# thegedge/StereoReconstruction

Hardware: AMD Instinct MI355X
Metric: Mdisparity-hypotheses/s (WxHxD) (higher is better)
Workload: dtype f64; 1 GPU; C3: synthetic rectified 1920x1080 pair, 256 depth levels, GeodesicWeight r=5; TwoView WTA both directions + cross-check; one pair per GPU; width=1920, height=1080, depth_levels=256, window_radius=5, weights=geodesic, pairs_per_gpu=1, pair_seed_rank0=1592590339, pair_seed_of_rank_r=seed + 0x10000*r, parallelism=single GPU

## Files before the change

stereoreconstruction_amd/csrc/srh_strip.hip:

```cpp
#include "srh_internal.hpp"
#include "srh_geom.hpp"
#include "srh_walk.hpp"

#include <type_traits>

namespace srh {

#ifdef SRH_EXPERIMENT
__device__ int g_strip_exp_repeat = 1;
void strip_exp_set(int repeat) { (void)hipMemcpyToSymbol(HIP_SYMBOL(g_strip_exp_repeat), &repeat, sizeof(int)); }
#endif

#define ST_TP 32
#define ST_NCB 8
#define ST_CHUNK 320
#define ST_BROWS 1

typedef __attribute__((address_space(3))) void st_lds_void;
typedef __attribute__((address_space(1))) const void st_gbl_void;
typedef __attribute__((address_space(3))) volatile int st_lds_vint;

__global__ void padded_plane_kernel(const double *__restrict__ gray_tv, int W, int H, double *__restrict__ out)
{
	const int SP = padded_stride(W), HP = H + 2*SRH_PADY;
	const size_t n = (size_t)SP*HP;
	const double nan = __builtin_nan("");
	for (size_t k = (size_t)blockIdx.x*blockDim.x + threadIdx.x; k < n; k += (size_t)gridDim.x*blockDim.x) {
		const int x = (int)(k % (size_t)SP) - SRH_PADL, y = (int)(k / (size_t)SP) - SRH_PADY;
		out[k] = (x >= 0 && y >= 0 && x < W && y < H) ? gray_tv[(size_t)y*W + x] : nan;
	}
}

void launch_padded_plane(hipStream_t st, const double *gray_tv, int w, int h, double *out) {
	size_t n = padded_size(w, h);
	size_t b = (n + 255)/256; if (b > 4096) b = 4096;
	hipLaunchKernelGGL(padded_plane_kernel, dim3((unsigned)b), dim3(256), 0, st, gray_tv, w, h, out);
}

__global__ void padded_full_kernel(const double *__restrict__ gray_tv, int W, int H, int R, uint8_t *__restrict__ out)
{
	const int SP = padded_stride(W), HP = H + 2*SRH_PADY;
	const size_t n = (size_t)SP*HP;
	for (size_t k = (size_t)blockIdx.x*blockDim.x + threadIdx.x; k < n; k += (size_t)gridDim.x*blockDim.x) {
		const int x = (int)(k % (size_t)SP) - SRH_PADL, y = (int)(k / (size_t)SP) - SRH_PADY;
		bool ok = x - R >= 0 && y - R >= 0 && x + R < W && y + R < H;
		for (int row = -R; ok && row <= R; ++row)
			for (int col = -R; col <= R; ++col) {
				const double v = gray_tv[(size_t)(y + row)*W + (x + col)];
				ok = ok && (v == v);
			}
		out[k] = ok ? 1 : 0;
	}
}

void launch_padded_full(hipStream_t st, const double *gray_tv, int w, int h, int R, uint8_t *out) {
	size_t n = padded_size(w, h);
	size_t b = (n + 255)/256; if (b > 4096) b = 4096;
	hipLaunchKernelGGL(padded_full_kernel, dim3((unsigned)b), dim3(256), 0, st, gray_tv, w, h, R, out);
}

__global__ void pixel_range_kernel(const ViewDev *__restrict__ views, int ref, int oth, srh_params P, int y0, int nrows,
                                   const double *__restrict__ tnum, int cstride, PixRange *__restrict__ prange)
{
	const ViewDev &L = views[ref];
	const int W = L.w;
	const size_t q = (size_t)blockIdx.x*blockDim.x + threadIdx.x;
	if (q >= (size_t)nrows*W) return;
	const int x = (int)(q % W), y = y0 + (int)(q / W);
	int lo = 0, hi = -1;
	if (L.mask[(size_t)y*W + x] == 1) {
		const Ray ray = cam_unproject(L.cam, (x + 0.5) / P.image_scale, (y + 0.5) / P.image_scale);
		pinhole_column_range(ray, L.cam, views[oth], P, tnum, cstride, lo, hi);
	}
	PixRange r; r.lo = lo; r.hi = hi;
	prange[q] = r;
}

void launch_pixel_range(hipStream_t st, const ViewDev *views, int ref, int oth, int width, const srh_params &P,
                        int y0, int nrows, const double *tnum, int cstride, PixRange *prange)
{
	const size_t n = (size_t)nrows*width;
	hipLaunchKernelGGL(pixel_range_kernel, dim3((unsigned)((n + 255)/256)), dim3(256), 0, st,
	                   views, ref, oth, P, y0, nrows, tnum, cstride, prange);
}

int strip_chunk_columns() { return ST_CHUNK; }

struct StripArgs {
	int W, H, y0, nrows;
	const double *wimg;
	const double *pconst;
	const PixRange *prange;
	const double *ref_tvp, *oth_tvp;
	const uint8_t *oth_fullp;
	double *cost; int cstride;
	Counters *cnt;
	int n1, n2;
	int nitems;
	double weight_cutoff, bad_ret, max_color_diff;
	CertBound cb;
	int redo;
};

static void strip_items(StripArgs &a) {
	a.n1 = ((a.nrows*3/4)/16)*16;
	a.n2 = a.n1 + (((a.nrows - a.n1)*2/3)/8)*8;
	const int nseg = a.n1/16 + (a.n2 - a.n1)/8 + (a.nrows - a.n2 + 3)/4;
	a.nitems = nseg*((a.W + ST_TP - 1)/ST_TP);
}

template <int R, int NBUF>
struct StripSmem {
	static constexpr int WS = 2*R + 1;
	static constexpr int T = WS*WS;
	static constexpr int WP = (WS + 1) & ~1;
	static constexpr int WPIX = WS*WP;
	static constexpr int RW = ST_CHUNK + 2*R + ST_NCB + 2;
	static constexpr int LW = (ST_TP + 2*R + 1) & ~1;
	static constexpr int NS = WS + 1;
	static constexpr int FW = (RW + 4 + 15) & ~15;
	static constexpr int NBMAX = ST_CHUNK/ST_NCB + 1;
	static constexpr int GL_CAP = 3072;
	static constexpr int GL_SINGLES = GL_CAP - ST_TP*NBMAX;
	alignas(16) double w[NBUF][WS][ST_TP][WP];
	alignas(16) double rt[NS][RW];
	alignas(16) double rto[NBUF == 2 ? NS : 1][RW];
	alignas(16) double lt[NS][LW];
	alignas(16) double pc[2][ST_TP][SRH_PC];
	alignas(16) PixRange pr[2][ST_TP];
	alignas(16) unsigned char full[2][FW];
	unsigned short glist[GL_CAP];
	int glist_n, gsingle_n;
	int item;
	unsigned long long badcols[ST_CHUNK/64 + 2];
	int simd[8];
	int prog[NBUF == 2 ? 8 : 1][64];
	static_assert(ST_CHUNK <= 512 && ST_TP <= 64, "work-list entry = pixel*512 + column in 16 bits");
	static_assert(RW % 2 == 0 && LW % 2 == 0 && WP % 2 == 0, "16-byte rows");
	static_assert(RW - R + 4 <= SRH_PADR + 1, "padded planes cover every staged piece");
};

__device__ __forceinline__ void st_dma16(const void *src, void *dst, int nbytes, int lane) {
	for (int off = 0; off < nbytes; off += 1024) {
		if (off + lane*16 < nbytes)
			__builtin_amdgcn_global_load_lds((st_gbl_void *)((const char *)src + off + lane*16),
			                                 (st_lds_void *)((char *)dst + off), 16, 0, 0);
	}
}
__device__ __forceinline__ void st_dma4(const void *src, void *dst, int nbytes, int lane) {
	for (int off = 0; off < nbytes; off += 256) {
		if (off + lane*4 < nbytes)
			__builtin_amdgcn_global_load_lds((st_gbl_void *)((const char *)src + off + lane*4),
			                                 (st_lds_void *)((char *)dst + off), 4, 0, 0);
	}
}

template <int R, int NBUF>
__device__ __noinline__ double strip_cost_general(const StripSmem<R, NBUF> &S, int wb, int s0, int i, int rc,
                                                  double weight_cutoff, double bad_ret, double max_color_diff)
{
	typedef StripSmem<R, NBUF> Smem;
	constexpr int WS = Smem::WS, NS = Smem::NS;
	double meanL = 0, meanR = 0, totalWeight = 0.0;
#pragma unroll 1
	for (int row = 0; row < WS; ++row) {
		const int sl = s0 + row >= NS ? s0 + row - NS : s0 + row;
		double gl[WS], gr[WS], wt[WS];
#pragma unroll
		for (int col = 0; col < WS; ++col) { gl[col] = S.lt[sl][i + col]; gr[col] = S.rt[sl][rc + col]; wt[col] = S.w[wb][row][i][col]; }
#pragma unroll
		for (int col = 0; col < WS; ++col) {
			const bool ok = gl[col] == gl[col] && gr[col] == gr[col] && wt[col] > weight_cutoff;
			const double pl = wt[col]*gl[col], pr = wt[col]*gr[col];
			meanL += ok ? pl : 0.0;
			meanR += ok ? pr : 0.0;
			totalWeight += ok ? wt[col] : 0.0;
		}
	}
	if (totalWeight < 1e-10) return bad_ret;
	meanL /= totalWeight;
	meanR /= totalWeight;
	double sum1 = 0, sum2 = 0, sum3 = 0;
#pragma unroll 1
	for (int row = 0; row < WS; ++row) {
		const int sl = s0 + row >= NS ? s0 + row - NS : s0 + row;
		double gl[WS], gr[WS], wt[WS];
#pragma unroll
		for (int col = 0; col < WS; ++col) { gl[col] = S.lt[sl][i + col]; gr[col] = S.rt[sl][rc + col]; wt[col] = S.w[wb][row][i][col]; }
#pragma unroll
		for (int col = 0; col < WS; ++col) {
			const bool ok = gl[col] == gl[col] && gr[col] == gr[col] && wt[col] > weight_cutoff;
			const double a = wt[col]*gl[col] - meanL;
			const double b = wt[col]*gr[col] - meanR;
			const double ab = a*b, aa = a*a, bb = b*b;
			sum1 += ok ? ab : 0.0;
			sum2 += ok ? aa : 0.0;
			sum3 += ok ? bb : 0.0;
		}
	}
	const double v = 255*(1.0 - fabs(sum1) / sqrt(sum2 * sum3));
	return (v < max_color_diff) ? v : max_color_diff;
}

template <int R, int NBUF>
__device__ __noinline__ void strip_select_block(const StripSmem<R, NBUF> &S, int wb, int s0, int pi, int rc, unsigned store,
                                                double *__restrict__ dst, double weight_cutoff, double bad_ret, double max_color_diff,
                                                int ra, int rb)
{
	typedef StripSmem<R, NBUF> Smem;
	constexpr int WS = Smem::WS, NS = Smem::NS, NCB = ST_NCB, NR = NCB + 2*R;
	double mLs[NCB], mRs[NCB], tws[NCB];
#pragma unroll
	for (int j = 0; j < NCB; ++j) { mLs[j] = 0.0; mRs[j] = 0.0; tws[j] = 0.0; }
#pragma unroll 1
	for (int row = ra; row < rb; ++row) {
		const int sl = s0 + row >= NS ? s0 + row - NS : s0 + row;
		double rr[NR], rv[NR];
		const double2 *rp = reinterpret_cast<const double2 *>((NBUF == 2 && (rc & 1)) ? &S.rto[sl][rc - 1] : &S.rt[sl][rc]);
#pragma unroll
		for (int m = 0; m < NR/2; ++m) { const double2 v = rp[m]; rr[2*m] = v.x; rr[2*m + 1] = v.y; }
#pragma unroll
		for (int m = 0; m < NR; ++m) { const bool okr = rr[m] == rr[m]; rv[m] = okr ? 1.0 : 0.0; rr[m] = okr ? rr[m] : 0.0; }
#pragma unroll
		for (int col = 0; col < WS; ++col) {
			const double gl = S.lt[sl][pi + col], wt = S.w[wb][row][pi][col];
			const bool okl = gl == gl && wt > weight_cutoff;
			const double w0 = okl ? wt : 0.0, pl0 = okl ? wt*gl : 0.0;
#pragma unroll
			for (int j = 0; j < NCB; ++j) {
				mLs[j] += pl0*rv[col + j];
				mRs[j] += w0*rr[col + j];
				tws[j] += w0*rv[col + j];
			}
		}
	}
#pragma unroll
	for (int j = 0; j < NCB; ++j) { mLs[j] /= tws[j]; mRs[j] /= tws[j]; }
	double s1[NCB], s2v[NCB], s3[NCB];
#pragma unroll
	for (int j = 0; j < NCB; ++j) { s1[j] = 0.0; s2v[j] = 0.0; s3[j] = 0.0; }
#pragma unroll 1
	for (int row = ra; row < rb; ++row) {
		const int sl = s0 + row >= NS ? s0 + row - NS : s0 + row;
		double rr[NR], rv[NR];
		const double2 *rp = reinterpret_cast<const double2 *>((NBUF == 2 && (rc & 1)) ? &S.rto[sl][rc - 1] : &S.rt[sl][rc]);
#pragma unroll
		for (int m = 0; m < NR/2; ++m) { const double2 v = rp[m]; rr[2*m] = v.x; rr[2*m + 1] = v.y; }
#pragma unroll
		for (int m = 0; m < NR; ++m) { const bool okr = rr[m] == rr[m]; rv[m] = okr ? 1.0 : 0.0; rr[m] = okr ? rr[m] : 0.0; }
#pragma unroll
		for (int col = 0; col < WS; ++col) {
			const double gl = S.lt[sl][pi + col], wt = S.w[wb][row][pi][col];
			const bool okl = gl == gl && wt > weight_cutoff;
			const double pl = wt*(gl == gl ? gl : 0.0), kl = okl ? 1.0 : 0.0;
#pragma unroll
			for (int j = 0; j < NCB; ++j) {
				const double k = kl*rv[col + j];
				const double a = (pl - mLs[j])*k, bq = (wt*rr[col + j] - mRs[j])*k;
				s1[j] += a*bq;
				s2v[j] += a*a;
				s3[j] += bq*bq;
			}
		}
	}
#pragma unroll
	for (int j = 0; j < NCB; ++j) {
		if ((store >> j) & 1u) {
			double result = bad_ret;
			if (!(tws[j] < 1e-10)) {
				const double v = 255*(1.0 - fabs(s1[j]) / sqrt(s2v[j] * s3[j]));
				result = (v < max_color_diff) ? v : max_color_diff;
			}
			dst[(ptrdiff_t)j*ST_TP] = result;
		}
	}
}

template <int R, int NWV, int NBUF, int AR, bool BORDER>
__global__ __launch_bounds__(NWV*64, 2)
void twoview_strip_cost_kernel(const StripArgs A)
{
	constexpr bool FMA = AR != 0, CERT = AR == 3 || AR == 5, ONEPASS = AR == 5;
	typedef StripSmem<R, NBUF> Smem;
	constexpr int WS = Smem::WS, WP = Smem::WP, WPIX = Smem::WPIX, RW = Smem::RW, LW = Smem::LW, NS = Smem::NS;
	constexpr int NCB = ST_NCB, CHUNK = ST_CHUNK;
	constexpr int NR = NCB + 2*R;
	constexpr int G = 2*NWV;
	constexpr int NT = NWV*64;
	constexpr bool PAD = NBUF == 1;
	static_assert(NR % 2 == 0, "16-byte rows");
	static_assert((NWV == 4 && NBUF == 1) || (NWV == 8 && NBUF == 2), "two forms");
	extern __shared__ __align__(16) unsigned char smem_raw[];
	Smem &S = *reinterpret_cast<Smem *>(smem_raw);
	const Smem &CS = S;

	const int tid = threadIdx.x;
	const int lane = tid & 63;
	const int wv = __builtin_amdgcn_readfirstlane(tid >> 6);
	const int pg = wv & 3;
	const int i = pg*8 + (lane & 7);
	const int g = (lane >> 3) + 8*(wv >> 2);
	const int W = A.W;
	const int tiles_per_row = (W + ST_TP - 1)/ST_TP;
	const int SP = padded_stride(W);
	unsigned n_dev = 0;
	int partner = wv;
	if (NWV == 8) {
		const int simd = (int)__builtin_amdgcn_s_getreg((1 << 11) | (4 << 6) | 4);
		if (lane == 0) S.simd[wv] = simd;
		S.prog[wv][lane] = 0;
		__syncthreads();
		for (int j = 0; j < NWV; ++j) if (j != wv && CS.simd[j] == simd) { partner = j; break; }
		partner = __builtin_amdgcn_readfirstlane(partner);
	}
	int prog = 0;
	auto prog_step = [&](int units, int &seen) {
		if (NWV == 8) {
			prog += units;
			*(st_lds_vint *)&S.prog[wv][lane] = prog;
			seen = *(st_lds_vint *)&S.prog[partner][lane];
		}
	};
	auto prog_yield = [&](int seen) {
		if (NWV == 8) {
			const int ps = __builtin_amdgcn_readfirstlane(seen), pm = __builtin_amdgcn_readfirstlane(prog);
			asm volatile("s_nop 0\n\ts_cmp_gt_i32 %0, %1\n\ts_cbranch_scc1 1f\n\ts_setprio 1\n\ts_branch 2f\n1:\n\ts_setprio 0\n2:"
			             :: "s"(pm), "s"(ps) : "scc");
		}
	};
#ifdef SRH_PROFILE_PHASES
	unsigned long long ph[8] = {0, 0, 0, 0, 0, 0, 0, 0};
	unsigned long long tp = __builtin_readcyclecounter();
	const unsigned long long t_begin = tp;
	unsigned long long n_tiles = 0, n_gen = 0;
#define ST_STAMP(k) do { const unsigned long long tn_ = __builtin_readcyclecounter(); ph[k] += tn_ - tp; tp = tn_; } while (0)
#else
#define ST_STAMP(k) do { } while (0)
#endif

	for (;;) {
		if (tid == 0) S.item = (int)atomicAdd(BORDER ? &A.cnt->strip_ticket_border : &A.cnt->strip_ticket, 1u);
		__syncthreads();
		const int item = __builtin_amdgcn_readfirstlane(S.item);
		ST_STAMP(0);
		if (item >= A.nitems) break;
		int seg = item / tiles_per_row, tx = item - seg*tiles_per_row;
		if (BORDER) {
			const int nseg = (A.n1 + ST_BROWS - 1)/ST_BROWS + (A.nrows - A.n2 + ST_BROWS - 1)/ST_BROWS;
			const int k = item / nseg;
			seg = item - k*nseg;
			tx = k == 0 ? 0 : k == 1 ? tiles_per_row - 1 : k - 1;
		}
		int ya, nh;
		if (BORDER) {
			const int st = (A.n1 + ST_BROWS - 1)/ST_BROWS;
			if (seg < st) { ya = seg*ST_BROWS; nh = A.n1 - ya; }
			else { ya = A.n2 + (seg - st)*ST_BROWS; nh = A.nrows - ya; }
			if (nh > ST_BROWS) nh = ST_BROWS;
		} else {
			const int s16 = A.n1 >> 4, s8 = (A.n2 - A.n1) >> 3;
			if (seg < s16) { ya = seg*16; nh = 16; }
			else if (seg < s16 + s8) { ya = A.n1 + (seg - s16)*8; nh = 8; }
			else { ya = A.n2 + (seg - s16 - s8)*4; nh = 4; }
			if (ya + nh > A.nrows) nh = A.nrows - ya;
		}
		const int x0 = tx*ST_TP;
		const int x = x0 + i;
		int cs = 0, rowbase = 0;

		auto issue_tile_inputs = [&](int r, int buf, int wb, bool consts, bool windows) {
			const size_t px0 = (size_t)r*W + x0;
			if (consts && wv == 0) st_dma16(A.pconst + px0*SRH_PC, &S.pc[buf][0][0], ST_TP*SRH_PC*8, lane);
			if (consts && wv == 1) st_dma4(A.prange + px0, &S.pr[buf][0], ST_TP*8, lane);
			if (windows) {
				const double *wt = A.wimg + ((size_t)r*tiles_per_row + tx)*(size_t)(ST_TP*WPIX);
				if (NBUF == 1) {
					for (int a = 0; a < WS; ++a)
						st_dma16(wt + (size_t)a*(ST_TP*WP) + pg*8*WP, &S.w[wb][a][pg*8][0], 8*WP*8, lane);
				} else {
					constexpr int NBYTES = ST_TP*WPIX*8;
					for (int off = wv*1024; off < NBYTES; off += NWV*1024)
						if (off + lane*16 < NBYTES)
							__builtin_amdgcn_global_load_lds((st_gbl_void *)((const char *)wt + off + lane*16),
							                                 (st_lds_void *)((char *)&S.w[wb][0][0][0] + off), 16, 0, 0);
				}
			}
		};
		auto issue_row = [&](int yy, int sl) {
			const double *src = A.oth_tvp + (size_t)(yy + SRH_PADY)*SP + (cs - R + SRH_PADL);
			if (wv < 3) { if (wv*1024 + lane*16 < RW*8) __builtin_amdgcn_global_load_lds((st_gbl_void *)((const char *)src + wv*1024 + lane*16),
			                                                                              (st_lds_void *)((char *)&S.rt[sl][0] + wv*1024), 16, 0, 0); }
			else if (wv == 3) st_dma16(A.ref_tvp + (size_t)(yy + SRH_PADY)*SP + (x0 - R + SRH_PADL), &S.lt[sl][0], LW*8, lane);
			else if (NBUF == 2 && wv < 7) {
				const int pc = wv - 4;
				if (pc*1024 + lane*16 < RW*8) __builtin_amdgcn_global_load_lds((st_gbl_void *)((const char *)(src + 1) + pc*1024 + lane*16),
				                                                                (st_lds_void *)((char *)&S.rto[sl][0] + pc*1024), 16, 0, 0);
			}
		};
		static_assert(RW*8 <= 3*1024, "three pieces per row of the other view");
		auto issue_full = [&](int fy, int fb) {
			const size_t a0 = (size_t)(fy + SRH_PADY)*SP + (size_t)(cs + SRH_PADL);
			if (!BORDER && wv == NWV - 1) st_dma4(A.oth_fullp + (a0 & ~(size_t)3), &S.full[fb][0], (RW + 4 + 3) & ~3, lane);
		};

		bool first = true;
		for (int r = ya; r < ya + nh; ++r) {
			const int y = A.y0 + r;
			const int cur = (r - ya) & 1, nxt = cur ^ 1;
			const int wcur = NBUF == 2 ? cur : 0, wnxt = NBUF == 2 ? nxt : 0;
			const bool has_next = r + 1 < ya + nh;
			if (first) issue_tile_inputs(r, cur, wcur, true, true);
			asm volatile("s_waitcnt vmcnt(0)" ::: "memory");
			ST_STAMP(1);
			__builtin_amdgcn_s_barrier();
			ST_STAMP(2);

			int cmin, cmax, cmin_raw;
			{
				const int pi = lane & 31;
				const PixRange q = CS.pr[cur][pi];
				int lo = q.lo, hi = q.hi;
				if (x0 + pi >= W) { lo = 0; hi = -1; }
				if (hi >= lo) hi = dense_cover_hi(lo, hi, NCB, G, PAD);
				int mn = hi >= lo ? lo : 2147483647, mx = hi >= lo ? hi : -2147483647;
#define ST_ROR(v, n) __builtin_amdgcn_update_dpp(0, (v), 0x120 + (n), 0xf, 0xf, false)
#pragma unroll
				for (int d = 8; d >= 1; d >>= 1) {
					const int on = d == 8 ? ST_ROR(mn, 8) : d == 4 ? ST_ROR(mn, 4) : d == 2 ? ST_ROR(mn, 2) : ST_ROR(mn, 1);
					const int ox = d == 8 ? ST_ROR(mx, 8) : d == 4 ? ST_ROR(mx, 4) : d == 2 ? ST_ROR(mx, 2) : ST_ROR(mx, 1);
					mn = on < mn ? on : mn; mx = ox > mx ? ox : mx;
				}
#undef ST_ROR
				{
					const int m0 = __builtin_amdgcn_readlane(mn, 0), m1 = __builtin_amdgcn_readlane(mn, 16);
					const int x0_ = __builtin_amdgcn_readlane(mx, 0), x1_ = __builtin_amdgcn_readlane(mx, 16);
					cmin_raw = m0 < m1 ? m0 : m1;
					cmax = x0_ > x1_ ? x0_ : x1_;
				}
				cmin = cmin_raw & ~1;
			}
			const bool any = cmin_raw <= cmax;
			if (first || (any && (cmin < cs || cmax > cs + CHUNK - 1))) {
				if (!first) __builtin_amdgcn_s_barrier();
				cs = any ? cmin : 0;
				rowbase = y - R;
				for (int rr = 0; rr < WS; ++rr) issue_row(y - R + rr, rr);
				issue_full(y, cur);
				asm volatile("s_waitcnt vmcnt(0)" ::: "memory");
				__builtin_amdgcn_s_barrier();
			}
			if (any && cmax > cs + CHUNK - 1) {
				if (tid == 0) atomicAdd(&A.cnt->strip_overflow, 1ull);
				cmax = cs + CHUNK - 1;
			}
			first = false;
			const int s0 = (y - R - rowbase) % NS;
			if (has_next) {
				issue_row(y + R + 1, (y + R + 1 - rowbase) % NS);
				issue_full(y + 1, nxt);
				issue_tile_inputs(r + 1, nxt, wnxt, true, NBUF == 2);
			}
			const int foff = BORDER ? 0 : (int)(((size_t)(y + SRH_PADY)*SP + (size_t)(cs + SRH_PADL)) & 3);
			const unsigned char *rfull = &CS.full[cur][foff];
			const int bra = BORDER ? (y < R ? R - y : 0) : 0;
			const int brb = BORDER ? (y + R > A.H - 2 ? WS - (y + R - (A.H - 2)) : WS) : WS;
			if (BORDER) {
				unsigned char *cok = &S.full[nxt][0];
				for (int k = tid; k < RW; k += NT) {
					bool ok = true;
					for (int row = bra; row < brb; ++row) {
						const int sl = s0 + row >= NS ? s0 + row - NS : s0 + row;
						const double v = CS.rt[sl][k];
						ok = ok && v == v;
					}
					cok[k] = ok ? 1 : 0;
				}
				if (g == 0) {
					bool all = x < W;
					double mL = 0, tw = 0;
					for (int row = bra; row < brb; ++row) {
						const int sl = s0 + row >= NS ? s0 + row - NS : s0 + row;
						for (int col = 0; col < WS; ++col) {
							const double gl = CS.lt[sl][i + col], wt = CS.w[wcur][row][i][col];
							all = all && gl == gl && wt > A.weight_cutoff;
							mL += wt*gl;
							tw += wt;
						}
					}
					double s2 = 0;
					if (all && !(tw < 1e-10)) {
						mL /= tw;
						for (int row = bra; row < brb; ++row) {
							const int sl = s0 + row >= NS ? s0 + row - NS : s0 + row;
							for (int col = 0; col < WS; ++col) {
								const double t = CS.w[wcur][row][i][col]*CS.lt[sl][i + col] - mL;
								s2 += t*t;
							}
						}
					} else all = false;
					S.pc[cur][i][0] = mL; S.pc[cur][i][1] = tw; S.pc[cur][i][2] = s2; S.pc[cur][i][3] = all ? 1.0/tw : 0.0;
				}
				__syncthreads();
				for (int k = tid; k < CHUNK + NCB; k += NT) {
					bool ok = true;
					for (int d = 0; d < WS; ++d) ok = ok && cok[k + d] != 0;
					S.full[cur][k] = ok ? 1 : 0;
				}
				__syncthreads();
			}

			bool need_general = false;
			{
				const int pi = lane & 31;
				const PixRange q = CS.pr[cur][pi];
				const bool live = x0 + pi < W && q.hi >= q.lo;
				bool bad = live && !(CS.pc[cur][pi][3] != 0.0);
#pragma unroll
				for (int it = 0; it < (CHUNK + 63)/64 + 1; ++it) {
					const int k = it*64 + lane, c = cs + k;
					const bool colbad = k < CHUNK + NCB && rfull[k] == 0;
					if (colbad && c >= cmin_raw && c <= cmax) bad = true;
					const unsigned long long m = __ballot(colbad);
					if (wv == 0 && lane == 0) S.badcols[it] = m;
				}
				need_general = __any(bad) != 0;
			}

			if (NWV == 8) { prog = 0; *(st_lds_vint *)&S.prog[wv][lane] = 0; __builtin_amdgcn_s_setprio(1); }
			int e_min, e_max;
			{
				const PixRange q = CS.pr[cur][i];
				e_min = q.lo; e_max = q.hi;
				if (x >= W) { e_min = 0; e_max = -1; }
				if (e_max >= e_min) e_max = dense_cover_hi(e_min, e_max, NCB, G, PAD);
			}
			const bool lall = CS.pc[cur][i][3] != 0.0;
			const double sig3 = CERT ? A.cb.sigma3(CS.pc[cur][i][2]) : 0.0;
			const bool pix_exact = CERT && A.redo && !(sig3 < __builtin_inf());
			const size_t tile = (size_t)r*tiles_per_row + tx;
			ST_STAMP(3);
			if (e_max >= e_min) {
				const int lo = e_min > cs ? e_min : cs;
				const int hi = e_max < cs + CHUNK - 1 ? e_max : cs + CHUNK - 1;
				const int lo_e = PAD ? (lo & ~1) : lo;
				const int nblocks = hi >= lo ? (hi - lo_e + NCB)/NCB : 0;
				double *crow = A.cost + tile*(size_t)A.cstride*ST_TP + i;
#ifdef SRH_EXPERIMENT
				const int exp_rep = g_strip_exp_repeat;
				for (int rep = 0; rep < exp_rep; ++rep)
#endif
				for (int b = g; b < (lall ? nblocks : 0); b += G) {
					const int c0 = lo_e + b*NCB;
					const int rc = c0 - cs;
					const double *rbase = (!PAD && (rc & 1)) ? &CS.rto[0][0] - 1 : &CS.rt[0][0];
					unsigned vm = 0;
#pragma unroll
					for (int j = 0; j < NCB; ++j) {
						const int c = c0 + j;
						vm |= (c >= lo && c <= hi && rfull[rc + j] != 0) ? 1u << j : 0u;
					}
					const bool fast = vm != 0;
					n_dev += __builtin_popcount(vm);
					bool bad_blk = false;
					auto two_sweeps = [&](auto fma_c, auto cert_c) {
						constexpr bool FMAc = decltype(fma_c)::value, CERTc = decltype(cert_c)::value;
						const double mL = CS.pc[cur][i][0], tw = CS.pc[cur][i][1], s2 = CS.pc[cur][i][2];
						const int ra = BORDER ? bra : 0, rb = BORDER ? brb : WS;
						const int sa = BORDER ? (s0 + ra >= NS ? s0 + ra - NS : s0 + ra) : s0;
						double r_[NR], wv_[WS], acc[NCB];
						{
							const double2 *rp = reinterpret_cast<const double2 *>(rbase + sa*RW + rc);
							const double2 *wp = reinterpret_cast<const double2 *>(&CS.w[wcur][ra][i][0]);
#pragma unroll
							for (int m = 0; m < NR/2; ++m) { const double2 v = rp[m]; r_[2*m] = v.x; r_[2*m + 1] = v.y; }
#pragma unroll
							for (int m = 0; m < (WS - 1)/2; ++m) { const double2 v = wp[m]; wv_[2*m] = v.x; wv_[2*m + 1] = v.y; }
							wv_[WS - 1] = CS.w[wcur][ra][i][WS - 1];
						}
#pragma unroll
						for (int j = 0; j < NCB; ++j) acc[j] = 0.0;
						__builtin_amdgcn_s_waitcnt(0xC07F);
#pragma unroll 1
						for (int row = ra; row < rb; ++row) {
							int seen = 0;
							prog_step(1, seen);
							const int nrow = row + 1 < rb ? row + 1 : ra;
							const int nsl = s0 + nrow >= NS ? s0 + nrow - NS : s0 + nrow;
							const double2 *rp = reinterpret_cast<const double2 *>(rbase + nsl*RW + rc);
							const double2 *wp = reinterpret_cast<const double2 *>(&CS.w[wcur][nrow][i][0]);
#pragma unroll
							for (int col = 0; col < WS; ++col) {
								if (FMAc) {
#pragma unroll
									for (int j = 0; j < NCB; ++j) acc[j] = __builtin_fma(wv_[col], r_[col + j], acc[j]);
								} else {
									double pr[NCB];
#pragma unroll
									for (int j = 0; j < NCB; ++j) pr[j] = wv_[col]*r_[col + j];
									__builtin_amdgcn_sched_barrier(0);
#pragma unroll
									for (int j = 0; j < NCB; ++j) acc[j] += pr[j];
								}
								__builtin_amdgcn_sched_barrier(0);
								if (col & 1) {
									const double2 v = rp[col >> 1]; r_[col - 1] = v.x; r_[col] = v.y;
									const double2 u = wp[col >> 1]; wv_[col - 1] = u.x; wv_[col] = u.y;
									__builtin_amdgcn_sched_barrier(0);
								}
							}
#pragma unroll
							for (int m = (WS - 1)/2; m < NR/2; ++m) { const double2 v = rp[m]; r_[2*m] = v.x; r_[2*m + 1] = v.y; }
							wv_[WS - 1] = CS.w[wcur][nrow][i][WS - 1];
							prog_yield(seen);
						}
						double mR[NCB], s1[NCB], s3[NCB], av[WS];
#pragma unroll
						for (int col = 0; col < WS; ++col) av[col] = CS.lt[sa][i + col];
#pragma unroll
						for (int j = 0; j < NCB; ++j) { mR[j] = acc[j]/tw; s1[j] = 0.0; s3[j] = 0.0; }
						__builtin_amdgcn_s_waitcnt(0xC07F);
#pragma unroll 1
						for (int row = ra; row < rb; ++row) {
							int seen = 0;
							prog_step(3, seen);
							const int nrow = row + 1 < rb ? row + 1 : ra;
							const int nsl = s0 + nrow >= NS ? s0 + nrow - NS : s0 + nrow;
							const double2 *rp = reinterpret_cast<const double2 *>(rbase + nsl*RW + rc);
							const double2 *wp = reinterpret_cast<const double2 *>(&CS.w[wcur][nrow][i][0]);
							const double *lp = &CS.lt[nsl][i];
#pragma unroll
							for (int col = 0; col < WS; ++col) {
								const double wt = wv_[col];
								if (FMAc) {
									const double a = __builtin_fma(wt, av[col], -mL);
									double bb[NCB];
#pragma unroll
									for (int j = 0; j < NCB; ++j) bb[j] = __builtin_fma(wt, r_[col + j], -mR[j]);
									__builtin_amdgcn_sched_barrier(0);
#pragma unroll
									for (int j = 0; j < NCB; ++j) { s1[j] = __builtin_fma(a, bb[j], s1[j]); s3[j] = __builtin_fma(bb[j], bb[j], s3[j]); }
								} else {
									double bb[NCB], u1[NCB], u3[NCB];
									const double pa = wt*av[col];
#pragma unroll
									for (int j = 0; j < NCB; ++j) bb[j] = wt*r_[col + j];
									__builtin_amdgcn_sched_barrier(0);
									const double a = pa - mL;
#pragma unroll
									for (int j = 0; j < NCB; ++j) bb[j] = bb[j] - mR[j];
									__builtin_amdgcn_sched_barrier(0);
#pragma unroll
									for (int j = 0; j < NCB; ++j) { u1[j] = a*bb[j]; u3[j] = bb[j]*bb[j]; }
									__builtin_amdgcn_sched_barrier(0);
#pragma unroll
									for (int j = 0; j < NCB; ++j) { s1[j] += u1[j]; s3[j] += u3[j]; }
								}
								__builtin_amdgcn_sched_barrier(0);
								av[col] = lp[col];
								if (col & 1) {
									const double2 v = rp[col >> 1]; r_[col - 1] = v.x; r_[col] = v.y;
									const double2 u = wp[col >> 1]; wv_[col - 1] = u.x; wv_[col] = u.y;
								}
								__builtin_amdgcn_sched_barrier(0);
							}
#pragma unroll
							for (int m = (WS - 1)/2; m < NR/2; ++m) { const double2 v = rp[m]; r_[2*m] = v.x; r_[2*m + 1] = v.y; }
							wv_[WS - 1] = CS.w[wcur][nrow][i][WS - 1];
							prog_yield(seen);
						}
#pragma unroll
						for (int j = 0; j < NCB; ++j) {
							const int c = c0 + j;
							if (c >= lo && c <= hi && rfull[rc + j] != 0) {
								const double v = 255*(1.0 - fabs(s1[j]) / sqrt(s2 * s3[j]));
								if (CERTc) {
									if (!(s3[j] >= sig3) && A.redo) bad_blk = true;
									crow[(size_t)(c - e_min)*ST_TP] = !(s3[j] >= sig3) ? __builtin_nan("") : (v > A.cb.m_hi ? A.max_color_diff : v);
								} else crow[(size_t)(c - e_min)*ST_TP] = (v < A.max_color_diff) ? v : A.max_color_diff;
							}
							__builtin_amdgcn_sched_barrier(0);
						}
					};
					if (BORDER) {
						if (fast) two_sweeps(std::false_type(), std::false_type());
					} else if (fast && ONEPASS && !pix_exact) {
						const double mL = CS.pc[cur][i][0], itw = CS.pc[cur][i][3], s2 = CS.pc[cur][i][2];
						double r_[NR], q_[NR], w_[WS], l_[WS], P_[NCB], Q_[NCB], U_[NCB];
						{
							const double2 *rp = reinterpret_cast<const double2 *>(rbase + s0*RW + rc);
							const double2 *wp = reinterpret_cast<const double2 *>(&CS.w[wcur][0][i][0]);
#pragma unroll
							for (int m = 0; m < NR/2; ++m) { const double2 v = rp[m]; r_[2*m] = v.x; r_[2*m + 1] = v.y; }
#pragma unroll
							for (int m = 0; m < (WS - 1)/2; ++m) { const double2 v = wp[m]; w_[2*m] = v.x; w_[2*m + 1] = v.y; }
							w_[WS - 1] = CS.w[wcur][0][i][WS - 1];
#pragma unroll
							for (int col = 0; col < WS; ++col) l_[col] = CS.lt[s0][i + col];
						}
#pragma unroll
						for (int j = 0; j < NCB; ++j) { P_[j] = 0.0; Q_[j] = 0.0; U_[j] = 0.0; }
						__builtin_amdgcn_s_waitcnt(0xC07F);
#pragma unroll 1
						for (int row = 0; row < WS; ++row) {
							int seen = 0;
							prog_step(4, seen);
							const int nrow = row + 1 < WS ? row + 1 : 0;
							const int nsl = s0 + nrow >= NS ? s0 + nrow - NS : s0 + nrow;
							const double2 *rp = reinterpret_cast<const double2 *>(rbase + nsl*RW + rc);
							const double2 *wp = reinterpret_cast<const double2 *>(&CS.w[wcur][nrow][i][0]);
							const double *lp = &CS.lt[nsl][i];
#pragma unroll
							for (int k = 0; k < NCB - 1; ++k) q_[k] = r_[k]*r_[k];
#pragma unroll
							for (int col = 0; col < WS; ++col) {
								q_[col + NCB - 1] = r_[col + NCB - 1]*r_[col + NCB - 1];
								const double a = __builtin_fma(w_[col], l_[col], -mL);
								const double c = a*w_[col], d = w_[col]*w_[col];
								__builtin_amdgcn_sched_barrier(0);
#pragma unroll
								for (int j = 0; j < NCB; ++j) P_[j] = __builtin_fma(w_[col], r_[col + j], P_[j]);
#pragma unroll
								for (int j = 0; j < NCB; ++j) Q_[j] = __builtin_fma(c, r_[col + j], Q_[j]);
#pragma unroll
								for (int j = 0; j < NCB; ++j) U_[j] = __builtin_fma(d, q_[col + j], U_[j]);
								__builtin_amdgcn_sched_barrier(0);
								l_[col] = lp[col];
								if (col & 1) {
									const double2 v = rp[col >> 1]; r_[col - 1] = v.x; r_[col] = v.y;
									const double2 u = wp[col >> 1]; w_[col - 1] = u.x; w_[col] = u.y;
								}
								__builtin_amdgcn_sched_barrier(0);
							}
#pragma unroll
							for (int m = (WS - 1)/2; m < NR/2; ++m) { const double2 v = rp[m]; r_[2*m] = v.x; r_[2*m + 1] = v.y; }
							w_[WS - 1] = CS.w[wcur][nrow][i][WS - 1];
							prog_yield(seen);
						}
						constexpr double TT = (double)(WS*WS);
						const double zmax2 = A.cb.zmax2, mhi = A.cb.m_hi, mcd = A.max_color_diff, SA = CS.pc[cur][i][4];
						const bool redo = A.redo != 0;
#pragma unroll
						for (int j = 0; j < NCB; ++j) {
							bool okc;
							const double v = onepass_finish(P_[j], Q_[j], U_[j], SA, itw, s2, TT, sig3, zmax2, okc);
							const bool st = (vm >> j) & 1u;
							bad_blk |= st & !okc & redo;
							if (st) crow[(size_t)(c0 + j - e_min)*ST_TP] = !okc ? __builtin_nan("") : (v > mhi ? mcd : v);
						}
					} else if (fast && !ONEPASS && !pix_exact) two_sweeps(std::integral_constant<bool, FMA>(), std::integral_constant<bool, CERT>());
					if (!BORDER && fast && CERT && (pix_exact || bad_blk)) two_sweeps(std::false_type(), std::false_type());
				}
			}
			if (NWV == 8) __builtin_amdgcn_s_setprio(2);
			ST_STAMP(4);
			if (need_general) {
				if (tid == 0) { S.glist_n = 0; S.gsingle_n = 0; }
				__syncthreads();
				for (int p = tid; p < ST_TP*Smem::NBMAX; p += NT) {
					const int pi = p / Smem::NBMAX, b = p % Smem::NBMAX;
					const PixRange q = CS.pr[cur][pi];
					int qlo = q.lo, qhi = q.hi;
					if (x0 + pi >= W) { qlo = 0; qhi = -1; }
					if (qhi >= qlo) qhi = dense_cover_hi(qlo, qhi, NCB, G, PAD);
					if (qhi > cs + CHUNK - 1) qhi = cs + CHUNK - 1;
					if (qhi < qlo) continue;
					const int c0 = (PAD ? (qlo & ~1) : qlo) + b*NCB;
					if (c0 > qhi) continue;
					const bool pall = CS.pc[cur][pi][3] != 0.0;
					unsigned need = 0xffu;
					if (qlo > c0) need &= 0xffu << (qlo - c0);
					if (c0 + NCB - 1 > qhi) need &= 0xffu >> (c0 + NCB - 1 - qhi);
					if (pall) {
						const int rc = c0 - cs, wd = rc >> 6, sh = rc & 63;
						unsigned long long bits = CS.badcols[wd] >> sh;
						if (sh) bits |= CS.badcols[wd + 1] << (64 - sh);
						need &= (unsigned)bits;
					}
					if (!need) continue;
					bool as_block = __builtin_popcount(need) == NCB;
					if (!as_block) {
						const int at = atomicAdd(&S.gsingle_n, __builtin_popcount(need));
						if (at + __builtin_popcount(need) <= Smem::GL_SINGLES) {
							int k = 0;
#pragma unroll
							for (int j = 0; j < NCB; ++j)
								if ((need >> j) & 1u) { S.glist[Smem::GL_CAP - 1 - (at + k)] = (unsigned short)(pi*512 + (c0 + j - cs)); ++k; }
						} else {
							for (int k = at; k < at + __builtin_popcount(need) && k < Smem::GL_SINGLES; ++k) S.glist[Smem::GL_CAP - 1 - k] = 0xffffu;
							as_block = true;
						}
					}
					if (as_block) S.glist[atomicAdd(&S.glist_n, 1)] = (unsigned short)(pi*64 + b);
				}
				__syncthreads();
				ST_STAMP(5);
#ifdef SRH_PROFILE_PHASES
				++n_gen;
#endif
				const int nblk = S.glist_n;
				const int nsingle = S.gsingle_n < Smem::GL_SINGLES ? S.gsingle_n : Smem::GL_SINGLES;
				for (int q = tid; q < nblk; q += NT) {
					const int pi = S.glist[q] >> 6, b = S.glist[q] & 63;
					const PixRange pq = CS.pr[cur][pi];
					int qhi = dense_cover_hi(pq.lo, pq.hi, NCB, G, PAD);
					if (qhi > cs + CHUNK - 1) qhi = cs + CHUNK - 1;
					const int c0 = (PAD ? (pq.lo & ~1) : pq.lo) + b*NCB;
					const bool pall = CS.pc[cur][pi][3] != 0.0;
					unsigned store = 0;
#pragma unroll
					for (int j = 0; j < NCB; ++j) {
						const int c = c0 + j;
						if (c >= pq.lo && c <= qhi && !(pall && rfull[c - cs])) { store |= 1u << j; ++n_dev; }
					}
					strip_select_block<R, NBUF>(CS, wcur, s0, pi, c0 - cs, store,
					                            A.cost + (tile*(size_t)A.cstride)*ST_TP + (ptrdiff_t)(c0 - pq.lo)*ST_TP + pi,
					                            A.weight_cutoff, A.bad_ret, A.max_color_diff,
					                            y < R ? R - y : 0, y + R > A.H - 2 ? WS - (y + R - (A.H - 2)) : WS);
				}
				ST_STAMP(6);
				for (int q = tid; q < nsingle; q += NT) {
					const unsigned short e = S.glist[Smem::GL_CAP - 1 - q];
					if (e == 0xffffu) continue;
					const int pi = e >> 9, k = e & 511;
					++n_dev;
					A.cost[(tile*(size_t)A.cstride + (size_t)(cs + k - CS.pr[cur][pi].lo))*ST_TP + pi] =
						strip_cost_general<R, NBUF>(CS, wcur, s0, pi, k, A.weight_cutoff, A.bad_ret, A.max_color_diff);
				}
				ST_STAMP(7);
				__syncthreads();
			}
			if (NBUF == 1 && has_next) issue_tile_inputs(r + 1, nxt, 0, false, true);
			ST_STAMP(2);
#ifdef SRH_PROFILE_PHASES
			++n_tiles;
#endif
		}
	}
	block_count_add(&A.cnt->n_eval_device, n_dev);
#ifdef SRH_PROFILE_PHASES
	if (lane == 0) {
		for (int k = 0; k < 8; ++k) atomicAdd(&A.cnt->dbg_phase[k], ph[k]);
		atomicAdd(&A.cnt->dbg_blocks, n_tiles);
		atomicAdd(&A.cnt->dbg_cycles, n_gen);
		for (int k = 0; k < 8; ++k) atomicAdd(&A.cnt->dbg_wave[8*k + (wv & 7)], ph[k]);
		atomicAdd(&A.cnt->dbg_total_cycles, (unsigned long long)(__builtin_readcyclecounter() - t_begin));
		atomicAdd(&A.cnt->dbg_waves, 1ull);
	}
#endif
#undef ST_STAMP
}

template <int R, int NWV, int NBUF, int AR, bool BORDER>
static void launch_strip_variant(hipStream_t st, const StripArgs &a, int num_cus)
{
	typedef StripSmem<R, NBUF> Smem;
	size_t lds = sizeof(Smem);
	(void)hipFuncSetAttribute((const void *)twoview_strip_cost_kernel<R, NWV, NBUF, AR, BORDER>,
	                          hipFuncAttributeMaxDynamicSharedMemorySize, (int)lds);
	int grid = num_cus*(NBUF == 2 ? 1 : 2);
	if (grid > a.nitems) grid = a.nitems;
	if (grid < 1) grid = 1;
	hipLaunchKernelGGL((twoview_strip_cost_kernel<R, NWV, NBUF, AR, BORDER>), dim3((unsigned)grid), dim3(NWV*64), lds, st, a);
}

template <int R, int NWV, int NBUF>
static void launch_strip_arith(hipStream_t st, const StripArgs &a, int num_cus, int arith)
{
	const int tiles_per_row = (a.W + ST_TP - 1)/ST_TP;
	const int t = std::min(std::max(R - a.y0, 0), a.nrows);
	const int b = std::min(std::max(a.H - 1 - R - a.y0, t), a.nrows);
	if (b > t) {
		StripArgs m = a;
		const size_t tiles = (size_t)t*tiles_per_row;
		m.y0 = a.y0 + t; m.nrows = b - t;
		m.wimg = a.wimg + tiles*(ST_TP*StripSmem<R, NBUF>::WPIX);
		m.pconst = a.pconst + (size_t)t*a.W*SRH_PC;
		m.prange = a.prange + (size_t)t*a.W;
		m.cost = a.cost + tiles*(size_t)a.cstride*ST_TP;
		strip_items(m);
		if (arith == 5) launch_strip_variant<R, NWV, NBUF, 5, false>(st, m, num_cus);
		else if (arith == 3) launch_strip_variant<R, NWV, NBUF, 3, false>(st, m, num_cus);
		else if (arith == 1) launch_strip_variant<R, NWV, NBUF, 1, false>(st, m, num_cus);
		else launch_strip_variant<R, NWV, NBUF, 0, false>(st, m, num_cus);
	}
	if (t > 0 || b < a.nrows) {
		StripArgs e = a;
		e.n1 = t; e.n2 = b;
		e.nitems = ((t + ST_BROWS - 1)/ST_BROWS + (a.nrows - b + ST_BROWS - 1)/ST_BROWS)*tiles_per_row;
		launch_strip_variant<R, NWV, NBUF, 0, true>(st, e, num_cus);
	}
}

int strip_block_lanes(int cstride, int form) {
	if (form == 4) return 8;
	if (form == 8) return 16;
	return cstride > 16*ST_NCB ? 16 : 8;
}

bool launch_twoview_strip_cost(hipStream_t st, const ViewDev *views, int ref, int oth, int width, int height,
                               const srh_params &P, int y0, int nrows, const double *wimg, const double *pconst,
                               const PixRange *prange, const double *ref_tvp, const double *oth_tvp,
                               const uint8_t *oth_fullp, double *cost, int cstride, Counters *cnt, int arith, int num_cus,
                               int lanes, bool raw)
{
	(void)views; (void)ref; (void)oth;
	StripArgs a;
	a.W = width; a.H = height; a.y0 = y0; a.nrows = nrows;
	a.wimg = wimg; a.pconst = pconst; a.prange = prange;
	a.ref_tvp = ref_tvp; a.oth_tvp = oth_tvp; a.oth_fullp = oth_fullp;
	a.cost = cost; a.cstride = cstride; a.cnt = cnt;
	a.weight_cutoff = P.weight_cutoff; a.bad_ret = P.bad_ret; a.max_color_diff = P.max_color_diff;
	a.cb = cert_bound(P);
	a.redo = raw ? 0 : 1;
	const bool wide = lanes == 16;
	switch (P.window_radius) {
	case 5:
		if (wide) launch_strip_arith<5, 8, 2>(st, a, num_cus, arith); else launch_strip_arith<5, 4, 1>(st, a, num_cus, arith);
		return true;
	case 2:
		if (wide) launch_strip_arith<2, 8, 2>(st, a, num_cus, arith); else launch_strip_arith<2, 4, 1>(st, a, num_cus, arith);
		return true;
	default: return false;
	}
}

}
```

Measured before the change: 46190 Mhyp/s.

## Handle few bad columns per pixel inline instead of building general work lists

Interior (non-border) tiles now count, per pixel, how many unusable columns fall in that pixel's disparity range. When every pixel has all-valid weights and at most NCB-1 bad columns, the idle half of the waves (or all waves when there are four) compute those costs directly through strip_cost_general, one candidate per lane. This skips the syncthreads-heavy work-list construction pass, which is now kept only for the heavier case. It adds per-pixel popcount and ballot work on every tile and a new path whose correctness depends on the lane-to-candidate mapping.

```diff
diff --git a/stereoreconstruction_amd/csrc/srh_strip.hip b/stereoreconstruction_amd/csrc/srh_strip.hip
--- a/stereoreconstruction_amd/csrc/srh_strip.hip
+++ b/stereoreconstruction_amd/csrc/srh_strip.hip
@@ -15,6 +15,7 @@
 #define ST_NCB 8
 #define ST_CHUNK 320
 #define ST_BROWS 1
+#define ST_SIDE_MAX (ST_NCB - 1)
 
 typedef __attribute__((address_space(3))) void st_lds_void;
 typedef __attribute__((address_space(1))) const void st_gbl_void;
@@ -132,7 +133,9 @@
 	unsigned short glist[GL_CAP];
 	int glist_n, gsingle_n;
 	int item;
+	static constexpr int NBW = (ST_CHUNK + 63)/64 + 1;
 	unsigned long long badcols[ST_CHUNK/64 + 2];
+	static_assert(NBW <= ST_CHUNK/64 + 2 && NBW*64 >= ST_CHUNK + ST_NCB, "badcols");
 	int simd[8];
 	int prog[NBUF == 2 ? 8 : 1][64];
 	static_assert(ST_CHUNK <= 512 && ST_TP <= 64, "work-list entry = pixel*512 + column in 16 bits");
@@ -153,6 +156,11 @@
 			__builtin_amdgcn_global_load_lds((st_gbl_void *)((const char *)src + off + lane*4),
 			                                 (st_lds_void *)((char *)dst + off), 4, 0, 0);
 	}
+}
+
+__device__ __forceinline__ unsigned long long st_bits(int a, int b) {
+	a = a < 0 ? 0 : a; b = b > 63 ? 63 : b;
+	return a <= b ? (~0ull >> (63 - b)) & (~0ull << a) : 0ull;
 }
 
 template <int R, int NBUF>
@@ -509,21 +517,41 @@
 				__syncthreads();
 			}
 
-			bool need_general = false;
-			{
+			int p2form = 0;
+			if (!BORDER) {
+				const int pi = lane & 31;
+				const PixRange q = CS.pr[cur][pi];
+				const bool live = x0 + pi < W && q.hi >= q.lo;
+				int ka = 0, kb = -1;
+				if (live) {
+					int h = dense_cover_hi(q.lo, q.hi, NCB, G, PAD);
+					if (h > cs + CHUNK - 1) h = cs + CHUNK - 1;
+					ka = q.lo - cs; kb = h - cs;
+				}
+				int nbad = 0;
+#pragma unroll
+				for (int it = 0; it < Smem::NBW; ++it) {
+					const int k = it*64 + lane;
+					const unsigned long long m = __ballot(k < CHUNK + NCB && rfull[k] == 0);
+					if (wv == 0 && lane == 0) S.badcols[it] = m;
+					nbad += __builtin_popcountll(m & st_bits(ka - it*64, kb - it*64));
+				}
+				const bool lists = live && (!(CS.pc[cur][pi][3] != 0.0) || nbad > ST_SIDE_MAX);
+				p2form = __any(lists) ? 2 : __any(nbad > 0) ? 1 : 0;
+			} else {
 				const int pi = lane & 31;
 				const PixRange q = CS.pr[cur][pi];
 				const bool live = x0 + pi < W && q.hi >= q.lo;
 				bool bad = live && !(CS.pc[cur][pi][3] != 0.0);
 #pragma unroll
-				for (int it = 0; it < (CHUNK + 63)/64 + 1; ++it) {
+				for (int it = 0; it < Smem::NBW; ++it) {
 					const int k = it*64 + lane, c = cs + k;
 					const bool colbad = k < CHUNK + NCB && rfull[k] == 0;
 					if (colbad && c >= cmin_raw && c <= cmax) bad = true;
 					const unsigned long long m = __ballot(colbad);
 					if (wv == 0 && lane == 0) S.badcols[it] = m;
 				}
-				need_general = __any(bad) != 0;
+				p2form = __any(bad) ? 2 : 0;
 			}
 
 			if (NWV == 8) { prog = 0; *(st_lds_vint *)&S.prog[wv][lane] = 0; __builtin_amdgcn_s_setprio(1); }
@@ -751,9 +779,44 @@
 					if (!BORDER && fast && CERT && (pix_exact || bad_blk)) two_sweeps(std::false_type(), std::false_type());
 				}
 			}
+			ST_STAMP(4);
+			if (!BORDER && p2form == 1 && (NWV == 4 || wv >= 4)) {
+				constexpr int ST_SIDE_G0 = NWV == 8 ? 8 : 0;
+				static_assert(ST_SIDE_G0 + ST_SIDE_MAX <= G, "one candidate per block lane");
+				if (NWV == 8) __builtin_amdgcn_s_setprio(0);
+				unsigned long long bm[Smem::NBW];
+#pragma unroll
+				for (int it = 0; it < Smem::NBW; ++it) {
+					const int k = it*64 + lane;
+					bm[it] = __ballot(k < CHUNK + NCB && rfull[k] == 0);
+				}
+				const PixRange q = CS.pr[cur][i];
+				int col = -1;
+				if (x < W && q.hi >= q.lo && g >= ST_SIDE_G0) {
+					int h = dense_cover_hi(q.lo, q.hi, NCB, G, PAD);
+					if (h > cs + CHUNK - 1) h = cs + CHUNK - 1;
+					const int ka = q.lo - cs, kb = h - cs;
+					int kk = g - ST_SIDE_G0;
+#pragma unroll
+					for (int it = 0; it < Smem::NBW; ++it) {
+						unsigned long long m = bm[it] & st_bits(ka - it*64, kb - it*64);
+						const int c = __builtin_popcountll(m);
+						if (col < 0 && kk < c) {
+							for (; kk > 0; --kk) m &= m - 1;
+							col = it*64 + __builtin_ctzll(m);
+						}
+						kk -= c;
+					}
+				}
+				if (col >= 0) {
+					++n_dev;
+					A.cost[(tile*(size_t)A.cstride + (size_t)(cs + col - q.lo))*ST_TP + i] =
+						strip_cost_general<R, NBUF>(CS, wcur, s0, i, col, A.weight_cutoff, A.bad_ret, A.max_color_diff);
+				}
+				ST_STAMP(7);
+			}
 			if (NWV == 8) __builtin_amdgcn_s_setprio(2);
-			ST_STAMP(4);
-			if (need_general) {
+			if (p2form == 2) {
 				if (tid == 0) { S.glist_n = 0; S.gsingle_n = 0; }
 				__syncthreads();
 				for (int p = tid; p < ST_TP*Smem::NBMAX; p += NT) {
```

Result: no change. 46220 Mhyp/s, median of 2 (+0.1%).
